# xyfJASON/ctrlora

Measured on NVIDIA B200. Metric: ddim_steps_per_sec, higher is better.
Workload: dtype fp16 (fp32 accumulate)

## Files before the change

### ctrlora_b200/_lib.py

```python
import ctypes as C
import os

_LIB_PATH = os.path.join(os.path.dirname(os.path.abspath(__file__)), "lib", "libctrlora_b200.so")
_lib = None

c_void_p, c_int, c_ll, c_float = C.c_void_p, C.c_int, C.c_longlong, C.c_float


class GemmArgs(C.Structure):
    _fields_ = [
        ("a", c_void_p), ("a_b", c_int), ("a_h", c_int), ("a_w", c_int), ("a_c", c_int), ("a_ld", c_ll),
        ("w", c_void_p), ("kh", c_int), ("kw", c_int), ("pad", c_int),
        ("a2", c_void_p), ("a2_c", c_int), ("a2_ld", c_ll), ("w2", c_void_p),
        ("n", c_int), ("block_n", c_int), ("geglu", c_int),
        ("out", c_void_p * 3), ("seg_width", c_int), ("transposed", c_int * 3),
        ("ldc", c_int), ("out_f32", c_int),
        ("bias", c_void_p), ("rowbias", c_void_p), ("rows_per_img", c_int), ("rowbias_ld", c_int),
        ("residual", c_void_p), ("ldr", c_int), ("residual_f32", c_int), ("out_scale", c_float),
        ("head_dim", c_int), ("tok_pad", c_int), ("bf16", c_int),
        ("split_k", c_int), ("splitk_ws", c_void_p), ("splitk_ws_bytes", c_ll),
        ("splitk_counters", c_void_p), ("splitk_counters_len", c_int),
        ("dup_out", c_void_p), ("dup_ld", c_int), ("force_single_cta", c_int),
    ]

# ... 16 lines not shown
_STATUS = {1: "bad argument", 2: "CUDA error", 3: "tensor-map encode error", 4: "unsupported"}


def lib_path():
    return _LIB_PATH


def load():
    global _lib
    if _lib is None:
        if not os.path.exists(_LIB_PATH):
            raise CtrloraError(
                f"{_LIB_PATH} is missing: run `python -m ctrlora_b200.build` (needs nvcc). "
                "ctrlora_b200 has no CPU or PyTorch fallback.")
        _lib = C.CDLL(_LIB_PATH)
        _declare(_lib)
    return _lib


_P, _I, _L, _F = c_void_p, c_int, c_ll, c_float
_ARGTYPES = {
    "ctrlora_gemm_f16": [_P, _P],
    "ctrlora_gemm_f16_simt": [_P, _P],
    "ctrlora_groupnorm_f16": [_P, _P],
    "ctrlora_layernorm_f16": [_P, _L, _P, _L, _I, _I, _P, _P, _F, _P],
    "ctrlora_attention_f16": [_P, _L, _P, _L, _P, _I, _P, _L, _P, _I, _I, _I, _I, _I, _P],
    "ctrlora_attention_bwd_f16": [_P, _L, _P, _L, _P, _L, _P, _L, _P, _L, _P, _P, _P, _L, _P, _L, _P, _L, _I, _I, _I, _I, _I, _P],
    "ctrlora_nchw_f32_to_nhwc_f16": [_P, _P, _I, _I, _I, _I, _P],
    "ctrlora_nhwc_to_nchw_f32": [_P, _I, _L, _P, _I, _I, _I, _P],
    "ctrlora_timestep_embedding": [_P, _P, _P, _I, _I, _P],
    "ctrlora_small_linear": [_P, _I, _P, _P, _P, _I, _I, _I, _I, _I, _I, _P],
    "ctrlora_upsample2x_f16": [_P, _P, _I, _I, _I, _I, _P],
    "ctrlora_im2col_s2_f16": [_P, _P, _I, _I, _I, _I, _P],
    "ctrlora_cast_transpose_f32_to_f16": [_P, _P, _L, _I, _I, _P],
    "ctrlora_transpose_f16": [_P, _P, _L, _I, _I, _P],
    "ctrlora_conv_dgrad_weight_f16": [_P, _P, _I, _I, _I, _P],
    "ctrlora_set_sm_limit": [_I],
    "ctrlora_ddim_update": [_P, _P, _P, _P, _P, _P, _P, _I, _I, _F, _F, _F, _F, _F, _F, _P],
    "ctrlora_wgrad_tn_f16": [_P, _L, _P, _L, _I, _I, _I, _P, _L, _F, _F, _P, _L, _P],
    "ctrlora_groupnorm_bwd_f16": [_P, _P, _P, _P, _L, _F, _P, _L, _F, _P, _L, _P, _P, _P],
    "ctrlora_layernorm_bwd_f16": [_P, _L, _P, _L, _P, _L, _I, _I, _P, _F, _P, _P, _P, _L, _P],
    "ctrlora_geglu_fwd_f16": [_P, _P, _L, _I, _P],
    "ctrlora_geglu_bwd_f16": [_P, _P, _P, _L, _I, _P],
    "ctrlora_colsum": [_P, _I, _L, _L, _I, _F, _P, _P],
    "ctrlora_image_colsum_f16": [_P, _L, _I, _I, _I, _P, _L, _P],
    "ctrlora_upsample2x_bwd_f16": [_P, _P, _I, _I, _I, _I, _P],
# ... 18 lines not shown


def _declare(lib):
    lib.ctrlora_abi_version.restype = c_int
    lib.ctrlora_last_cuda_error.restype = C.c_char_p
    for name in EXPORTS:
        fn = getattr(lib, name)
        if name not in ("ctrlora_abi_version", "ctrlora_last_cuda_error"):
            fn.restype = c_int
            fn.argtypes = _ARGTYPES[name]


def check(status, what):
    if status != 0:
        err = load().ctrlora_last_cuda_error()
        raise CtrloraError(f"{what} failed: {_STATUS.get(status, status)} ({err.decode() if err else ''})")


EXPORTS = [
    "ctrlora_abi_version",
    "ctrlora_last_cuda_error",
    "ctrlora_gemm_f16",
    "ctrlora_gemm_f16_simt",
    "ctrlora_groupnorm_f16",
    "ctrlora_layernorm_f16",
    "ctrlora_attention_f16",
    "ctrlora_nchw_f32_to_nhwc_f16",
    "ctrlora_nhwc_to_nchw_f32",
    "ctrlora_timestep_embedding",
    "ctrlora_small_linear",
    "ctrlora_upsample2x_f16",
    "ctrlora_im2col_s2_f16",
    "ctrlora_cast_transpose_f32_to_f16",
    "ctrlora_transpose_f16",
    "ctrlora_conv_dgrad_weight_f16",
    "ctrlora_set_sm_limit",
    "ctrlora_ddim_update",
    "ctrlora_wgrad_tn_f16",
    "ctrlora_attention_bwd_f16",
    "ctrlora_groupnorm_bwd_f16",
    "ctrlora_layernorm_bwd_f16",
    "ctrlora_geglu_fwd_f16",
    "ctrlora_geglu_bwd_f16",
    "ctrlora_colsum",
    "ctrlora_image_colsum_f16",
    "ctrlora_upsample2x_bwd_f16",
# ... 19 lines not shown
```

### ctrlora_b200/csrc/common.cuh

```cuda
#pragma once
#include <cuda.h>
#include <cuda_runtime.h>
#include <cuda_fp16.h>
#include <stdint.h>
#include <stdio.h>
#include <stdlib.h>
#include <string.h>

#define CTRLORA_OK 0
#define CTRLORA_ERR_ARG 1
#define CTRLORA_ERR_CUDA 2
#define CTRLORA_ERR_TMAP 3
#define CTRLORA_ERR_UNSUPPORTED 4

namespace ctrl {

__device__ __forceinline__ uint32_t smem_u32(const void* p) {
    return static_cast<uint32_t>(__cvta_generic_to_shared(p));
}

__device__ __forceinline__ void mbar_init(uint64_t* bar, uint32_t count) {
    asm volatile("mbarrier.init.shared::cta.b64 [%0], %1;" ::"r"(smem_u32(bar)), "r"(count) : "memory");
}
__device__ __forceinline__ void fence_barrier_init() {
// ... 238 lines not shown
    const float e = fast_exp2(-z * z);
    const float t = fast_rcp(fmaf(0.27273706287f, fabsf(z), 1.0f));
    float poly = fmaf(1.061405429f, t, -1.453152027f);
    poly = fmaf(poly, t, 1.421413741f);
    poly = fmaf(poly, t, -0.284496736f);
    poly = fmaf(poly, t, 0.254829592f);
    const float w = poly * t * e;
    return fmaf(-0.5f * fabsf(x), w, fmaxf(x, 0.0f));
}

}

namespace ctrl {
constexpr uint32_t kPeerBitMask = 0xFEFFFFFFu;

__device__ __forceinline__ uint32_t cluster_ctarank() {
    uint32_t r;
    asm volatile("mov.u32 %0, %%cluster_ctarank;" : "=r"(r));
    return r;
}
__device__ __forceinline__ void cluster_sync_all() {
    asm volatile("barrier.cluster.arrive.release.aligned;\n\tbarrier.cluster.wait.acquire.aligned;" ::: "memory");
}
__device__ __forceinline__ void tma_load_3d_2cta(void* dst, const CUtensorMap* m, uint64_t* bar, int c0, int c1, int c2) {
    asm volatile(
        "cp.async.bulk.tensor.3d.cta_group::2.shared::cluster.global.mbarrier::complete_tx::bytes [%0], [%1, {%3, %4, %5}], [%2];" ::"r"(
            smem_u32(dst)),
        "l"(reinterpret_cast<uint64_t>(m)), "r"(smem_u32(bar) & kPeerBitMask), "r"(c0), "r"(c1), "r"(c2)
        : "memory");
}
__device__ __forceinline__ void tma_load_4d_2cta(void* dst, const CUtensorMap* m, uint64_t* bar, int c0, int c1, int c2, int c3) {
    asm volatile(
        "cp.async.bulk.tensor.4d.cta_group::2.shared::cluster.global.mbarrier::complete_tx::bytes [%0], [%1, {%3, %4, %5, %6}], "
        "[%2];" ::"r"(smem_u32(dst)),
        "l"(reinterpret_cast<uint64_t>(m)), "r"(smem_u32(bar) & kPeerBitMask), "r"(c0), "r"(c1), "r"(c2), "r"(c3)
        : "memory");
}
__device__ __forceinline__ void umma_f16_2cta(uint32_t d_tmem, uint64_t a_desc, uint64_t b_desc, uint32_t idesc, uint32_t accumulate) {
    asm volatile(
        "{\n\t.reg .pred p;\n\t"
        "setp.ne.b32 p, %4, 0;\n\t"
        "tcgen05.mma.cta_group::2.kind::f16 [%0], %1, %2, %3, p;\n\t}" ::"r"(d_tmem),
        "l"(a_desc), "l"(b_desc), "r"(idesc), "r"(accumulate)
        : "memory");
}
__device__ __forceinline__ void umma_commit_2cta(uint64_t* bar) {
// ... 165 lines not shown
```

### ctrlora_b200/csrc/gemm_sm100.cu

```cuda
#include "gemm_sm100.cuh"
#include "ctrlora_b200.h"
#include <stdio.h>
#include <string.h>

namespace ctrl {

__device__ __forceinline__ uint32_t pack_h2(float a, float b) {
    __half2 h = __floats2half2_rn(a, b);
    return *reinterpret_cast<uint32_t*>(&h);
}

template <bool GEGLU>
__device__ __forceinline__ void epilogue_chunk(const GemmKParams& p, float* v, const float* g, int c, int bn_out, int n0,
                                               bool row_ok, long long m, int img, int tok, const float* sb,
                                               const uint4* rpre = nullptr) {
    const int nbase = n0 + c;
    const bool full_chunk = (c + 32 <= bn_out) && (nbase + 32 <= p.N);
#pragma unroll
    for (int q = 0; q < 8; ++q) {
        const float4 b4 = lds128f(smem_u32(sb + c + 4 * q));
        v[4 * q] += b4.x; v[4 * q + 1] += b4.y; v[4 * q + 2] += b4.z; v[4 * q + 3] += b4.w;
    }
    if (GEGLU) {
#pragma unroll
// ... 94 lines not shown
            for (int j = 0; j < 32; ++j)
                if (c + j < bn_out && nbase + j < p.N) o[j] = __float2half_rn(v[j]);
        }
    }
}

__device__ __forceinline__ void red_add_v4(float* addr, float a, float b, float c, float d) {
    asm volatile("red.global.add.v4.f32 [%0], {%1, %2, %3, %4};" ::"l"(addr), "f"(a), "f"(b), "f"(c), "f"(d) : "memory");
}

template <bool GEGLU, bool PAIR>
__global__ void __launch_bounds__(GEMM_THREADS, 1)
gemm_tcgen05_kernel(const __grid_constant__ CUtensorMap tmA, const __grid_constant__ CUtensorMap tmB,
                    const __grid_constant__ CUtensorMap tmA2, const __grid_constant__ CUtensorMap tmB2,
                    const __grid_constant__ GemmEpiMaps em, const __grid_constant__ GemmKParams p) {
    extern __shared__ uint8_t smem_raw[];
    uint8_t* smem = reinterpret_cast<uint8_t*>((reinterpret_cast<uintptr_t>(smem_raw) + 1023) & ~uintptr_t(1023));
    uint64_t* bars = reinterpret_cast<uint64_t*>(smem + GEMM_SMEM_DATA);
    uint64_t* full = bars;
    uint64_t* empty = bars + GEMM_MAX_STAGES;
    uint64_t* tfull = bars + 2 * GEMM_MAX_STAGES;
    uint64_t* tempty = bars + 2 * GEMM_MAX_STAGES + 2;
    uint32_t* tmem_ptr = reinterpret_cast<uint32_t*>(bars + 2 * GEMM_MAX_STAGES + 4);
    volatile int* last_flag = reinterpret_cast<volatile int*>(bars + 2 * GEMM_MAX_STAGES + 5);
    uint64_t* rfull = bars + 2 * GEMM_MAX_STAGES + 6;
    uint64_t* rempty = bars + 2 * GEMM_MAX_STAGES + 8;
    float* sbias_all = reinterpret_cast<float*>(smem + GEMM_SMEM_DATA + 512);

    pdl_launch_dependents();
    const int warp = uniform_warp_idx();
    const int lane = threadIdx.x & 31;
    const int nstages = p.stages;
    const uint32_t rank = PAIR ? cluster_ctarank() : 0u;
    const bool leader = rank == 0;

    if (warp == 0 && lane == 0) {
        tma_prefetch_desc(&tmA);
        tma_prefetch_desc(&tmB);
        if (p.epi_tma) {
            tma_prefetch_desc(&em.out[0][0]);
            tma_prefetch_desc(&em.out[0][1]);
            if (p.epi_res) { tma_prefetch_desc(&em.res[0]); tma_prefetch_desc(&em.res[1]); }
        }
        if (p.kchunks2 > 0) {
            tma_prefetch_desc(&tmA2);
            tma_prefetch_desc(&tmB2);
        }
    }
    if (warp == 1 && lane == 0) {
        for (int i = 0; i < nstages; ++i) {
            mbar_init(&full[i], 1);
            mbar_init(&empty[i], 1);
        }
        for (int i = 0; i < 2; ++i) {
            mbar_init(&tfull[i], 1);
            mbar_init(&tempty[i], PAIR ? 2 * GEMM_EPI_WARPS : GEMM_EPI_WARPS);
            mbar_init(&rfull[i], 1);
// ... 2 lines not shown
        fence_barrier_init();
    }
    if (warp == 2) {
        if (PAIR) tmem_alloc_2cta(tmem_ptr, 512);
        else tmem_alloc(tmem_ptr, 512);
    }
    tc_fence_before();
    __syncthreads();
    if (PAIR) cluster_sync_all();
    tc_fence_after();
    const uint32_t tmem_base = *tmem_ptr;
    pdl_wait();

    const int m_tiles = p.tiles_w * p.tiles_h * p.tiles_b;
    const int m_units = PAIR ? (m_tiles + 1) / 2 : m_tiles;
    const int total_tiles = m_units * p.n_tiles * p.splits;
    const int tile_first = PAIR ? static_cast<int>(blockIdx.x >> 1) : static_cast<int>(blockIdx.x);
    const int tile_stride = PAIR ? static_cast<int>(gridDim.x >> 1) : static_cast<int>(gridDim.x);
    const int main_iters = p.taps * p.kchunks;
    const int k_iters = main_iters + p.kchunks2;
    const int bn_out = GEGLU ? (p.BN >> 1) : p.BN;

    auto decode = [&](int tile, int& mt, int& ks, int& nt) {
        mt = tile % m_units;
        if (PAIR) mt = 2 * mt + static_cast<int>(rank);
        const int rest = tile / m_units;
        ks = rest % p.splits;
        nt = rest / p.splits;
    };

    if (warp == 0) {
        {
            const uint32_t tx_bytes = PAIR ? 2 * (GEMM_A_BYTES + (p.BN >> 1) * 128) : GEMM_A_BYTES + p.BN * 128;
            const int kchunks = p.kchunks, kw = p.kw, pad = p.pad, kps = p.kiters_per_split;
            const uint32_t stage_bytes = static_cast<uint32_t>(p.stage_bytes);
            const uint32_t smem0 = smem_u32(smem), full0 = smem_u32(full), empty0 = smem_u32(empty);
            const uint32_t gate_off = GEMM_A_BYTES + static_cast<uint32_t>(bn_out) * 128;
            const uint32_t rfull0 = smem_u32(rfull), rempty0 = smem_u32(rempty);
            int stage = 0, rbuf = 0;
            uint32_t phase = 0, a_dst = smem0, fb = full0, eb = empty0, rphase = 0;
            for (int tile = tile_first; tile < total_tiles; tile += tile_stride) {
                int mt, ks, nt;
                decode(tile, mt, ks, nt);
                const int tw = mt % p.tiles_w, th = (mt / p.tiles_w) % p.tiles_h, tb = mt / (p.tiles_w * p.tiles_h);
                const int w0 = tw * p.bw - pad, h0 = th * p.bh - pad, b0 = tb * p.nb, n0 = nt * bn_out;
                const int brow = !PAIR ? n0 : GEGLU ? (leader ? n0 : p.N + n0) : n0 + static_cast<int>(rank) * (p.BN >> 1);
// ... 32 lines not shown
                        tma_load_3d_a<PAIR>(a_dst + GEMM_A_BYTES, &tmB2, fb, c0, 0, brow);
                    }
                    __syncwarp();
                    c0 += GEMM_BK;
                    a_dst += stage_bytes; fb += 8; eb += 8;
                    if (++stage == nstages) { stage = 0; phase ^= 1; a_dst = smem0; fb = full0; eb = empty0; }
                }
                if (p.epi_res) {
                    mbar_wait_a(rempty0 + 8 * rbuf, rphase ^ 1);
                    if (elect_one()) {
                        const uint32_t rb = rfull0 + 8 * rbuf;
                        const uint32_t dst = smem0 + p.epi_off + rbuf * p.epi_buf_bytes;
                        mbar_expect_tx_a(rb, GEMM_BM * bn_out * 2);
                        for (int b = 0; b < p.epi_nfull; ++b)
                            tma_load_4d_a<false>(dst + b * 16384, &em.res[0], rb, n0 + 64 * b, w0 + pad, h0 + pad, b0);
                        if (p.epi_tail)
                            tma_load_4d_a<false>(dst + p.epi_nfull * 16384, &em.res[1], rb, n0 + 64 * p.epi_nfull, w0 + pad, h0 + pad, b0);
                    }
                    __syncwarp();
                    if (++rbuf == p.epi_nbuf) { rbuf = 0; rphase ^= 1; }
                }
            }
        }
    } else if (warp == 1) {
        if (leader) {
            const int kps = p.kiters_per_split;
            const uint32_t idesc = p.idesc;
            const uint32_t full0 = smem_u32(full), empty0 = smem_u32(empty), tfull0 = smem_u32(tfull), tempty0 = smem_u32(tempty);
            const uint64_t a_desc0 = umma_desc_kmajor_sw128(smem_u32(smem));
            const uint64_t b_desc0 = umma_desc_kmajor_sw128(smem_u32(smem) + GEMM_A_BYTES);
            const uint32_t stage_step = static_cast<uint32_t>(p.stage_bytes) >> 4;
            int stage = 0;
            uint32_t phase = 0, fb = full0, eb = empty0, desc_off = 0;
            int acc = 0;
            uint32_t acc_phase = 0;
            for (int tile = tile_first; tile < total_tiles; tile += tile_stride) {
                const int ks = (tile / m_units) % p.splits;
                const int it0 = ks * kps, it1 = min(k_iters, it0 + kps);
                mbar_wait_a(tempty0 + 8 * acc, acc_phase ^ 1);
                tc_fence_after();
                const uint32_t d_tmem = tmem_base + acc * 256;
                uint32_t accum = 0;
                for (int it = it0; it < it1; ++it) {
                    mbar_wait_a(fb, phase);
                    tc_fence_after();
                    const uint64_t a_desc = a_desc0 + desc_off, b_desc = b_desc0 + desc_off;
                    if (elect_one()) {
#pragma unroll
                        for (int k = 0; k < GEMM_BK / 16; ++k) {
                            if (PAIR) umma_f16_2cta(d_tmem, a_desc + 2 * k, b_desc + 2 * k, idesc, (accum | k) ? 1u : 0u);
                            else umma_f16(d_tmem, a_desc + 2 * k, b_desc + 2 * k, idesc, (accum | k) ? 1u : 0u);
                        }
                        umma_commit_a<PAIR>(eb);
                        if (it + 1 == it1) umma_commit_a<PAIR>(tfull0 + 8 * acc);
                    }
                    __syncwarp();
                    accum = 1;
                    fb += 8; eb += 8; desc_off += stage_step;
                    if (++stage == nstages) { stage = 0; phase ^= 1; fb = full0; eb = empty0; desc_off = 0; }
                }
                acc ^= 1;
                if (acc == 0) acc_phase ^= 1;
            }
        }
    } else {
        const int lane_grp = warp & 3;
        const int half = (warp - 2) >> 2;
        const int r = lane_grp * 32 + lane;
        const int iw = r % p.bw, ih = (r / p.bw) % p.bh, ib = r / (p.bw * p.bh);
        int acc = 0;
        uint32_t acc_phase = 0;
        int tile_iter = 0;
        for (int tile = tile_first; tile < total_tiles; tile += tile_stride, ++tile_iter) {
            int mt, ks, nt;
            decode(tile, mt, ks, nt);
            const int tw = mt % p.tiles_w, th = (mt / p.tiles_w) % p.tiles_h, tb = mt / (p.tiles_w * p.tiles_h);
            const int gw = tw * p.bw + iw, gh = th * p.bh + ih, gb = tb * p.nb + ib;
            const bool row_ok = gw < p.W && gh < p.H && gb < p.Bn;
            const long long m = (static_cast<long long>(gb) * p.H + gh) * p.W + gw;
            const int n0 = nt * bn_out;
            const int img = row_ok ? static_cast<int>(m / p.rows_per_img) : 0;
            const int tok = row_ok ? static_cast<int>(m % p.rows_per_img) : 0;

            float* sb = sbias_all + (tile_iter & 1) * 512;
            {
                const int e = threadIdx.x - 64;
                float bv = 0.f, bg = 0.f;
// ... 127 lines not shown
                for (int i = 0; i < 4; ++i) {
                    const int c = 32 * half + 64 * i;
                    if (c >= bn_out) break;
                    uint32_t raw[32];
                    float v[32], g[GEGLU ? 32 : 1];
                    tmem_ld_32x32(t_row + c, raw);
                    if (GEGLU) {
                        uint32_t graw[32];
                        tmem_ld_32x32(t_row + bn_out + c, graw);
                        tmem_ld_wait();
#pragma unroll
                        for (int j = 0; j < 32; ++j) g[j] = __uint_as_float(graw[j]);
                    } else {
                        tmem_ld_wait();
                    }
#pragma unroll
                    for (int j = 0; j < 32; ++j) v[j] = __uint_as_float(raw[j]);
                    epilogue_chunk<GEGLU>(p, v, g, c, bn_out, n0, row_ok, m, img, tok, sb);
                }
                tc_fence_before();
                __syncwarp();
                if (lane == 0) { if (PAIR) mbar_arrive_leader(&tempty[acc]); else mbar_arrive(&tempty[acc]); }
            } else {
                const int tile_mn = nt * m_tiles + mt;
                const long long slice = static_cast<long long>(GEMM_BM) * p.BN;
                float* wrow0 = p.ws + static_cast<long long>(tile_mn) * p.splits * slice + static_cast<long long>(r) * 4;
                float* wrow = wrow0 + ks * slice;
                auto wofs = [](int col) { return static_cast<long long>(col >> 2) * (GEMM_BM * 4); };
                for (int c = 32 * half; c < p.BN; c += 64) {
                    uint32_t raw[32];
                    tmem_ld_32x32(t_row + c, raw);
                    tmem_ld_wait();
#pragma unroll
                    for (int q = 0; q < 8; ++q)
                        if (c + 4 * q < p.BN)
                            __stcg(reinterpret_cast<float4*>(wrow + wofs(c + 4 * q)),
                                   make_float4(__uint_as_float(raw[4 * q]), __uint_as_float(raw[4 * q + 1]),
                                               __uint_as_float(raw[4 * q + 2]), __uint_as_float(raw[4 * q + 3])));
                }
                tc_fence_before();
                __syncwarp();
                if (lane == 0) mbar_arrive(&tempty[acc]);
                __threadfence();
                asm volatile("bar.sync 1, %0;" ::"n"(32 * GEMM_EPI_WARPS) : "memory");
                if (warp == 2 && lane == 0) {
                    const unsigned int old = atomicAdd(&p.counters[tile_mn], 1u);
                    const int last = (old == static_cast<unsigned int>(p.splits - 1));
                    if (last) p.counters[tile_mn] = 0;
                    *last_flag = last;
                }
                asm volatile("bar.sync 1, %0;" ::"n"(32 * GEMM_EPI_WARPS) : "memory");
                const int is_last = *last_flag;
                if (is_last) {
                    __threadfence();
                    for (int c = 32 * half; c < bn_out; c += 64) {
                        float v[32], g[32];
#pragma unroll
                        for (int q = 0; q < 8; ++q) {
                            float4 t4 = make_float4(0.f, 0.f, 0.f, 0.f), g4 = t4;
                            if (c + 4 * q < bn_out) {
                                for (int sl = 0; sl < p.splits; ++sl) {
                                    const float4 x4 = __ldcg(reinterpret_cast<const float4*>(wrow0 + sl * slice + wofs(c + 4 * q)));
                                    t4.x += x4.x; t4.y += x4.y; t4.z += x4.z; t4.w += x4.w;
                                    if (GEGLU) {
                                        const float4 y4 = __ldcg(reinterpret_cast<const float4*>(wrow0 + sl * slice + wofs(bn_out + c + 4 * q)));
                                        g4.x += y4.x; g4.y += y4.y; g4.z += y4.z; g4.w += y4.w;
                                    }
                                }
                            }
                            v[4 * q] = t4.x; v[4 * q + 1] = t4.y; v[4 * q + 2] = t4.z; v[4 * q + 3] = t4.w;
                            g[4 * q] = g4.x; g[4 * q + 1] = g4.y; g[4 * q + 2] = g4.z; g[4 * q + 3] = g4.w;
                        }
                        epilogue_chunk<GEGLU>(p, v, g, c, bn_out, n0, row_ok, m, img, tok, sb);
                    }
                }
                asm volatile("bar.sync 1, %0;" ::"n"(32 * GEMM_EPI_WARPS) : "memory");
            }
            acc ^= 1;
            if (acc == 0) acc_phase ^= 1;
        }
        if (p.epi_tma && lane == 0) bulk_wait_group<0>();
    }
    tc_fence_before();
    __syncthreads();
    if (PAIR) cluster_sync_all();
    if (warp == 2) {
        __syncwarp();
        if (PAIR) tmem_dealloc_2cta(tmem_base, 512);
        else tmem_dealloc(tmem_base, 512);
    }
}

typedef CUresult (*PFN_tmapEncodeTiled)(CUtensorMap*, CUtensorMapDataType, cuuint32_t, void*, const cuuint64_t*,
                                        const cuuint64_t*, const cuuint32_t*, const cuuint32_t*, CUtensorMapInterleave,
                                        CUtensorMapSwizzle, CUtensorMapL2promotion, CUtensorMapFloatOOBfill);

PFN_tmapEncodeTiled get_tmap_encoder() {
    static PFN_tmapEncodeTiled fn = nullptr;
    if (!fn) {
// ... 24 lines not shown
    CUresult r = enc(map, CU_TENSOR_MAP_DATA_TYPE_FLOAT16, rank, const_cast<void*>(base), gdim, gstr, bx, es,
                     CU_TENSOR_MAP_INTERLEAVE_NONE, swz, CU_TENSOR_MAP_L2_PROMOTION_L2_256B,
                     CU_TENSOR_MAP_FLOAT_OOB_FILL_NONE);
    if (r != CUDA_SUCCESS) {
        fprintf(stderr, "ctrlora: cuTensorMapEncodeTiled failed (%d) rank %d dims", (int)r, rank);
        for (int i = 0; i < rank; ++i) fprintf(stderr, " %llu", (unsigned long long)dims[i]);
        fprintf(stderr, " box");
        for (int i = 0; i < rank; ++i) fprintf(stderr, " %u", box[i]);
        fprintf(stderr, "\n");
        return CTRLORA_ERR_TMAP;
    }
    return CTRLORA_OK;
}

static int pow2_floor(int x) {
    int p = 1;
    while (p * 2 <= x) p *= 2;
    return p;
}

static int g_num_sms = 0;
static int g_sm_limit = 0;
static bool g_attr_set = false;

}

using namespace ctrl;

extern "C" int ctrlora_gemm_f16(const ctrlora_gemm_args* a, void* stream_) {
    cudaStream_t stream = reinterpret_cast<cudaStream_t>(stream_);
    if (!a || !a->a || !a->w || !a->out[0]) return CTRLORA_ERR_ARG;
    if (a->a_c % 8 != 0 || a->a_ld % 8 != 0) return CTRLORA_ERR_ARG;
    if (a->kh != a->kw || (a->kh != 1 && a->kh != 3)) return CTRLORA_ERR_UNSUPPORTED;
    if (a->bf16) return CTRLORA_ERR_UNSUPPORTED;
    GemmKParams p;
    memset(&p, 0, sizeof(p));
    p.W = a->a_w; p.H = a->a_h; p.Bn = a->a_b;
    p.bw = pow2_floor(p.W < 128 ? p.W : 128);
    p.bh = pow2_floor(p.H < 128 / p.bw ? p.H : 128 / p.bw);
    p.nb = 128 / (p.bw * p.bh);
    p.tiles_w = (p.W + p.bw - 1) / p.bw;
    p.tiles_h = (p.H + p.bh - 1) / p.bh;
    p.tiles_b = (p.Bn + p.nb - 1) / p.nb;
    p.N = a->n;
    p.taps = a->kh * a->kw; p.kw = a->kw; p.pad = a->pad;
    p.kchunks = (a->a_c + GEMM_BK - 1) / GEMM_BK;
// ... 16 lines not shown
    const bool pair_ok = pair_env && pair_shape && g_num_sms >= 2 && a->force_single_cta == 0;
    static int epi_env = -1;
    if (epi_env < 0) {
        const char* e = getenv("CTRLORA_GEMM_EPI");
        epi_env = (e && e[0] == '0') ? 0 : (e && e[0] == '2') ? 2 : 1;
    }
    bool epi_legal = !a->out_f32 && a->split_k <= 1 && a->ldc % 8 == 0 && (reinterpret_cast<uintptr_t>(a->out[0]) & 15) == 0 &&
                     (!a->residual || (!a->residual_f32 && a->ldr % 8 == 0 && (reinterpret_cast<uintptr_t>(a->residual) & 15) == 0));
    if (a->seg_width > 0) {
        const int nseg = (a->n + a->seg_width - 1) / a->seg_width;
        if (a->residual || nseg > 3 || a->seg_width % 8 != 0) epi_legal = false;
        for (int i = 0; i < nseg && i < 3; ++i)
            if (!a->transposed[i] && (!a->out[i] || (reinterpret_cast<uintptr_t>(a->out[i]) & 15) != 0)) epi_legal = false;
        if (a->dup_out && ((reinterpret_cast<uintptr_t>(a->dup_out) & 15) != 0 || a->dup_ld % 8 != 0)) epi_legal = false;
    } else if (a->transposed[0] || a->dup_out) {
        epi_legal = false;
    }
    static int epi_kmax = -1;
    if (epi_kmax < 0) {
        const char* e = getenv("CTRLORA_GEMM_EPI_KMAX");
        epi_kmax = e ? atoi(e) : 32;
    }
    const bool epi_wanted = epi_legal && (epi_env == 2 || (epi_env == 1 && k_iters <= epi_kmax));
    int bn_out = a->block_n, splits = a->split_k > 0 ? a->split_k : 1;
    if (bn_out <= 0) {
        double best_cost = -1;
        const int max_out = p.geglu ? 128 : 256;
        static const int split_cands[] = {1, 2, 3, 4, 6, 8, 12, 16};
        for (int cand = max_out; cand >= 16; cand -= 16) {
            if (a->seg_width > 0 && a->seg_width % cand != 0) continue;
            if (epi_wanted && cand % 32 != 0) continue;
            const int bnt = p.geglu ? 2 * cand : cand;
            const int nt = (p.N + cand - 1) / cand;
            const long tiles_mn = (long)m_tiles * nt;
            const double waste = (double)nt * cand / p.N;
            for (int si = 0; si < 8; ++si) {
                int S = split_cands[si];
                if (a->split_k > 0) { if (si > 0) break; S = a->split_k; }
                if (S > 1) {
                    if (a->split_k <= 0) break;
                    if (!a->splitk_ws || !a->splitk_counters) break;
                    if ((long long)tiles_mn * S * GEMM_BM * bnt * 4 > a->splitk_ws_bytes || tiles_mn > a->splitk_counters_len) break;
                    if (a->seg_width > 0 && a->transposed[0] + a->transposed[1] + a->transposed[2] > 0 && false) break;
                }
                const int kps = (k_iters + S - 1) / S;
                if (S > 1 && kps < 4 && a->split_k <= 0) break;
                const int s_eff = (k_iters + kps - 1) / kps;
                const bool cpair = pair_ok && s_eff == 1 && bnt % 32 == 0;
                const long tiles = cpair ? (long)((m_tiles + 1) / 2) * nt : tiles_mn * s_eff;
                const long slots = cpair ? g_num_sms / 2 : g_num_sms;
                const long waves = (tiles + slots - 1) / slots;
                const double t_mma = kps * 4.0 * (bnt / 2 > 32 ? bnt / 2 : 32);
                const double t_load = kps * (double)(GEMM_A_BYTES + (cpair ? bnt / 2 : bnt) * 128) / 69.0;
                const double t_epi = (cand / 32 + 1) * 350.0;
                double t_tile = (t_mma > t_load ? t_mma : t_load);
                if (t_epi > t_tile) t_tile = t_epi;
                t_tile += 600.0;
                if (s_eff > 1) t_tile += bnt * 12.0 + t_epi;
                const double cost = waves * t_tile * (0.5 + 0.5 * waste);
                if (best_cost < 0 || cost < best_cost) { best_cost = cost; bn_out = cand; splits = s_eff; }
            }
        }
    }
    if (bn_out % 16 != 0 || bn_out < 16 || bn_out > (p.geglu ? 128 : 256)) return CTRLORA_ERR_ARG;
    if (a->seg_width > 0 && a->seg_width % bn_out != 0) return CTRLORA_ERR_ARG;
    p.BN = p.geglu ? 2 * bn_out : bn_out;
    p.n_tiles = (p.N + bn_out - 1) / bn_out;
    p.kiters_per_split = (k_iters + splits - 1) / splits;
    p.splits = (k_iters + p.kiters_per_split - 1) / p.kiters_per_split;
    if (p.splits > 1) {
        const long long tiles_mn = (long long)m_tiles * p.n_tiles;
        if (!a->splitk_ws || !a->splitk_counters || tiles_mn * p.splits * GEMM_BM * p.BN * 4 > a->splitk_ws_bytes ||
            tiles_mn > a->splitk_counters_len)
            return CTRLORA_ERR_ARG;
        p.ws = a->splitk_ws;
        p.counters = a->splitk_counters;
    }
    const bool pair = pair_ok && p.splits == 1 && (p.BN % 32 == 0);
    const int b_rows = pair ? p.BN / 2 : p.BN;
    p.stage_bytes = GEMM_A_BYTES + ((b_rows * 128 + 1023) / 1024) * 1024;
    int ring_bytes = GEMM_SMEM_DATA;
    {
        if (epi_wanted && p.splits == 1 && bn_out % 32 == 0) {
            const int nfull = bn_out / 64, tail = (bn_out % 64) ? 1 : 0;
            const int buf_bytes = nfull * 16384 + tail * 8192;
            int nbuf = 2;
            if ((GEMM_SMEM_DATA - 2 * buf_bytes) / p.stage_bytes < 3) nbuf = 1;
            static int nbuf_env = -1;
            if (nbuf_env < 0) {
                const char* e = getenv("CTRLORA_GEMM_EPI_NBUF");
                nbuf_env = e ? atoi(e) : 0;
            }
            if (nbuf_env == 1) nbuf = 1;
            if ((GEMM_SMEM_DATA - nbuf * buf_bytes) / p.stage_bytes >= 3) {
                p.epi_tma = 1; p.epi_nbuf = nbuf; p.epi_res = a->residual ? 1 : 0;
                p.epi_nfull = nfull; p.epi_tail = tail; p.epi_buf_bytes = buf_bytes;
                p.epi_off = GEMM_SMEM_DATA - nbuf * buf_bytes;
                ring_bytes = p.epi_off;
            }
        }
// ... 59 lines not shown
            box[0] = 32;
            return make_tmap_f16_sw(&dst[1], base, 4, dims, str, box, CU_TENSOR_MAP_SWIZZLE_64B);
        };
        if (a->seg_width > 0) {
            const int nseg = (p.N + a->seg_width - 1) / a->seg_width;
            for (int i = 0; i < nseg; ++i) {
                if (a->transposed[i]) continue;
                int rc = pair_of(em.out[i], a->out[i], a->ldc, a->seg_width, sw, sh, sb);
                if (rc) return rc;
            }
            if (a->dup_out) {
                int rc = pair_of(em.dup, a->dup_out, a->dup_ld, a->seg_width, sw, sh, sb);
                if (rc) return rc;
            }
        } else {
            int rc = pair_of(em.out[0], a->out[0], a->ldc, p.N, sw, sh, sb);
            if (rc) return rc;
        }
        if (p.epi_res) {
            int rc = pair_of(em.res, a->residual, a->ldr, p.N, p.bw, p.bh, p.nb);
            if (rc) return rc;
        }
    }
    if (!g_attr_set) {
        if (cudaFuncSetAttribute(gemm_tcgen05_kernel<false, false>, cudaFuncAttributeMaxDynamicSharedMemorySize, GEMM_SMEM_BYTES) != cudaSuccess ||
            cudaFuncSetAttribute(gemm_tcgen05_kernel<true, false>, cudaFuncAttributeMaxDynamicSharedMemorySize, GEMM_SMEM_BYTES) != cudaSuccess ||
            cudaFuncSetAttribute(gemm_tcgen05_kernel<false, true>, cudaFuncAttributeMaxDynamicSharedMemorySize, GEMM_SMEM_BYTES) != cudaSuccess ||
            cudaFuncSetAttribute(gemm_tcgen05_kernel<true, true>, cudaFuncAttributeMaxDynamicSharedMemorySize, GEMM_SMEM_BYTES) != cudaSuccess)
            return CTRLORA_ERR_CUDA;
        g_attr_set = true;
    }
    cudaError_t lrc;
    if (pair) {
        const int units = ((m_tiles + 1) / 2) * p.n_tiles;
        int clusters = (g_sm_limit > 0 && g_sm_limit < g_num_sms ? g_sm_limit : g_num_sms) / 2;
        if (units < clusters) clusters = units;
        const dim3 grid2(2 * clusters), block(GEMM_THREADS);
        lrc = p.geglu ? launch_cluster(gemm_tcgen05_kernel<true, true>, grid2, block, (size_t)GEMM_SMEM_BYTES, stream, 2u, tmA, tmB, tmA2, tmB2, em, p)
                      : launch_cluster(gemm_tcgen05_kernel<false, true>, grid2, block, (size_t)GEMM_SMEM_BYTES, stream, 2u, tmA, tmB, tmA2, tmB2, em, p);
    } else {
        const int total = m_tiles * p.n_tiles * p.splits;
        const int sms_avail = g_sm_limit > 0 && g_sm_limit < g_num_sms ? g_sm_limit : g_num_sms;
        const int grid = total < sms_avail ? total : sms_avail;
        lrc = p.geglu ? launch_pdl(gemm_tcgen05_kernel<true, false>, dim3(grid), dim3(GEMM_THREADS), (size_t)GEMM_SMEM_BYTES,
                                   stream, tmA, tmB, tmA2, tmB2, em, p)
                      : launch_pdl(gemm_tcgen05_kernel<false, false>, dim3(grid), dim3(GEMM_THREADS), (size_t)GEMM_SMEM_BYTES,
                                   stream, tmA, tmB, tmA2, tmB2, em, p);
    }
    if (lrc != cudaSuccess) return CTRLORA_ERR_CUDA;
    return cudaGetLastError() == cudaSuccess ? CTRLORA_OK : CTRLORA_ERR_CUDA;
}

extern "C" int ctrlora_set_sm_limit(int limit) {
    if (limit < 0) return CTRLORA_ERR_ARG;
    g_sm_limit = limit;
    return CTRLORA_OK;
}
```

### ctrlora_b200/csrc/gemm_sm100.cuh

```cuda
#pragma once
#include "common.cuh"

namespace ctrl {

constexpr int GEMM_BM = 128;
constexpr int GEMM_BK = 64;
constexpr int GEMM_MAX_STAGES = 10;
constexpr int GEMM_A_BYTES = GEMM_BM * GEMM_BK * 2;
constexpr int GEMM_EPI_WARPS = 8;
constexpr int GEMM_THREADS = 64 + 32 * GEMM_EPI_WARPS;
constexpr int GEMM_SMEM_DATA = 216 * 1024;
constexpr int GEMM_SMEM_BYTES = GEMM_SMEM_DATA + 1024  + 512  + 4096 ;

struct GemmEpiMaps {
    CUtensorMap out[3][2];
    CUtensorMap dup[2];
    CUtensorMap res[2];
};

struct GemmKParams {
    int W, H, Bn;
    int bw, bh, nb;
    int tiles_w, tiles_h, tiles_b;
    int N;
    int BN;
    int n_tiles;
    int taps, kw, pad;
    int kchunks;
    int kchunks2;
    int geglu;
    int stages, stage_bytes;
    int splits, kiters_per_split;
    float* ws;
    unsigned int* counters;
    uint32_t idesc;
    void* out[3];
    int seg_width;
    int transposed[3];
    int ldc;
    int out_f32;
    const float* bias;
    const float* rowbias;
    int rows_per_img;
    int rowbias_ld;
    int residual_f32;
    const __half* residual;
    int ldr;
    float out_scale;
    int head_dim, tok_pad;
    __half* dup_out;
    int dup_ld;
    int bf16;
    int epi_tma, epi_nbuf, epi_res;
    int epi_off, epi_buf_bytes;
    int epi_nfull, epi_tail;
};

// ... 2 lines not shown
```

### include/ctrlora_b200.h

```cpp
#ifndef CTRLORA_B200_H
#define CTRLORA_B200_H

#ifdef __cplusplus
extern "C" {
#endif

#define CTRLORA_ABI_VERSION 2

#define CTRLORA_STATUS_OK 0
#define CTRLORA_STATUS_BAD_ARGUMENT 1
#define CTRLORA_STATUS_CUDA_ERROR 2
#define CTRLORA_STATUS_TENSORMAP_ERROR 3
#define CTRLORA_STATUS_UNSUPPORTED 4

int ctrlora_abi_version(void);
const char* ctrlora_last_cuda_error(void);

int ctrlora_memset_zero(void* ptr, long long bytes, void* stream);

typedef struct ctrlora_gemm_args {
    const void* a;
    int a_b, a_h, a_w, a_c;
    long long a_ld;
    const void* w;
// ... 11 lines not shown
    int ldc;
    int out_f32;
    const float* bias;
    const float* rowbias;
    int rows_per_img;
    int rowbias_ld;
    const void* residual;
    int ldr;
    int residual_f32;
    float out_scale;
    int head_dim, tok_pad;
    int bf16;
    int split_k;
    float* splitk_ws;
    long long splitk_ws_bytes;
    unsigned int* splitk_counters;
    int splitk_counters_len;
    void* dup_out;
    int dup_ld;
    int force_single_cta;
} ctrlora_gemm_args;

int ctrlora_gemm_f16(const ctrlora_gemm_args* args, void* stream);

int ctrlora_gemm_f16_simt(const ctrlora_gemm_args* args, void* stream);

typedef struct ctrlora_groupnorm_args {
    const void* x1; const void* add1; float add1_scale; int c1; long long ld1;
    const void* x2; const void* add2; float add2_scale; int c2; long long ld2;
    int batch, hw, groups;
    const float* gamma; const float* beta; float eps; int silu;
    void* y;
    void* raw_out;
    void* stats_ws;
    int stats_prezeroed;
    float* partial_ws;
    long long partial_ws_floats;
    unsigned int* partial_counters;
    int partial_counters_len;
} ctrlora_groupnorm_args;
int ctrlora_groupnorm_f16(const ctrlora_groupnorm_args* args, void* stream);

int ctrlora_layernorm_f16(const void* x, long long ldx, void* y, long long ldy, int rows, int cols,
                          const float* gamma, const float* beta, float eps, void* stream);

int ctrlora_attention_f16(const void* q, long long ldq, const void* k, long long ldk, const void* vt, int nk_pad,
// ... 81 lines not shown
```

Baseline: 69.35.

## Replace global-workspace split-K with cluster-based DSMEM split-K reduction

Split-K partial sums are now exchanged through distributed shared memory inside a thread-block cluster of size `splits`. Each CTA reduces its share of rows and runs the epilogue for them, replacing the global workspace with its atomic counters and last-CTA reduction. The tile heuristic now considers split-K by default, even without a caller-supplied workspace, when the MN tile count underfills the SMs and the clusters fit in occupancy. This targets small-M/N, large-K GEMMs that leave SMs idle. The cost is extra cluster barriers and launch constraints, plus a new query export for the last chosen config.

```diff
diff --git a/ctrlora_b200/_lib.py b/ctrlora_b200/_lib.py
--- a/ctrlora_b200/_lib.py
+++ b/ctrlora_b200/_lib.py
@@ -62,6 +62,7 @@
 _ARGTYPES = {
     "ctrlora_gemm_f16": [_P, _P],
     "ctrlora_gemm_f16_simt": [_P, _P],
+    "ctrlora_gemm_last_config": [_P, _P, _P],
     "ctrlora_groupnorm_f16": [_P, _P],
     "ctrlora_layernorm_f16": [_P, _L, _P, _L, _I, _I, _P, _P, _F, _P],
     "ctrlora_attention_f16": [_P, _L, _P, _L, _P, _I, _P, _L, _P, _I, _I, _I, _I, _I, _P],
@@ -126,6 +127,7 @@
     "ctrlora_last_cuda_error",
     "ctrlora_gemm_f16",
     "ctrlora_gemm_f16_simt",
+    "ctrlora_gemm_last_config",
     "ctrlora_groupnorm_f16",
     "ctrlora_layernorm_f16",
     "ctrlora_attention_f16",
diff --git a/ctrlora_b200/csrc/common.cuh b/ctrlora_b200/csrc/common.cuh
--- a/ctrlora_b200/csrc/common.cuh
+++ b/ctrlora_b200/csrc/common.cuh
@@ -284,6 +284,14 @@
 __device__ __forceinline__ void cluster_sync_all() {
     asm volatile("barrier.cluster.arrive.release.aligned;\n\tbarrier.cluster.wait.acquire.aligned;" ::: "memory");
 }
+__device__ __forceinline__ uint32_t mapa_shared(uint32_t addr, uint32_t rank) {
+    uint32_t r;
+    asm volatile("mapa.shared::cluster.u32 %0, %1, %2;" : "=r"(r) : "r"(addr), "r"(rank));
+    return r;
+}
+__device__ __forceinline__ void st_dsmem128(uint32_t cluster_addr, uint32_t a, uint32_t b, uint32_t c, uint32_t d) {
+    asm volatile("st.shared::cluster.v4.b32 [%0], {%1, %2, %3, %4};" ::"r"(cluster_addr), "r"(a), "r"(b), "r"(c), "r"(d) : "memory");
+}
 __device__ __forceinline__ void tma_load_3d_2cta(void* dst, const CUtensorMap* m, uint64_t* bar, int c0, int c1, int c2) {
     asm volatile(
         "cp.async.bulk.tensor.3d.cta_group::2.shared::cluster.global.mbarrier::complete_tx::bytes [%0], [%1, {%3, %4, %5}], [%2];" ::"r"(
diff --git a/ctrlora_b200/csrc/gemm_sm100.cu b/ctrlora_b200/csrc/gemm_sm100.cu
--- a/ctrlora_b200/csrc/gemm_sm100.cu
+++ b/ctrlora_b200/csrc/gemm_sm100.cu
@@ -140,7 +140,6 @@
     uint64_t* tfull = bars + 2 * GEMM_MAX_STAGES;
     uint64_t* tempty = bars + 2 * GEMM_MAX_STAGES + 2;
     uint32_t* tmem_ptr = reinterpret_cast<uint32_t*>(bars + 2 * GEMM_MAX_STAGES + 4);
-    volatile int* last_flag = reinterpret_cast<volatile int*>(bars + 2 * GEMM_MAX_STAGES + 5);
     uint64_t* rfull = bars + 2 * GEMM_MAX_STAGES + 6;
     uint64_t* rempty = bars + 2 * GEMM_MAX_STAGES + 8;
     float* sbias_all = reinterpret_cast<float*>(smem + GEMM_SMEM_DATA + 512);
@@ -151,6 +150,7 @@
     const int nstages = p.stages;
     const uint32_t rank = PAIR ? cluster_ctarank() : 0u;
     const bool leader = rank == 0;
+    const bool csplit = !PAIR && p.splits > 1;
 
     if (warp == 0 && lane == 0) {
         tma_prefetch_desc(&tmA);
@@ -199,6 +199,13 @@
     const int bn_out = GEGLU ? (p.BN >> 1) : p.BN;
 
     auto decode = [&](int tile, int& mt, int& ks, int& nt) {
+        if (csplit) {
+            ks = tile % p.splits;
+            const int t = tile / p.splits;
+            mt = t % m_tiles;
+            nt = t / m_tiles;
+            return;
+        }
         mt = tile % m_units;
         if (PAIR) mt = 2 * mt + static_cast<int>(rank);
         const int rest = tile / m_units;
@@ -277,6 +284,7 @@
                 }
             }
         }
+        if (csplit) { cluster_sync_all(); cluster_sync_all(); }
     } else if (warp == 1) {
         if (leader) {
             const int kps = p.kiters_per_split;
@@ -290,7 +298,8 @@
             int acc = 0;
             uint32_t acc_phase = 0;
             for (int tile = tile_first; tile < total_tiles; tile += tile_stride) {
-                const int ks = (tile / m_units) % p.splits;
+                int mt, ks, nt;
+                decode(tile, mt, ks, nt);
                 const int it0 = ks * kps, it1 = min(k_iters, it0 + kps);
                 mbar_wait_a(tempty0 + 8 * acc, acc_phase ^ 1);
                 tc_fence_after();
@@ -318,6 +327,7 @@
                 if (acc == 0) acc_phase ^= 1;
             }
         }
+        if (csplit) { cluster_sync_all(); cluster_sync_all(); }
     } else {
         const int lane_grp = warp & 3;
         const int half = (warp - 2) >> 2;
@@ -491,59 +501,53 @@
                 __syncwarp();
                 if (lane == 0) { if (PAIR) mbar_arrive_leader(&tempty[acc]); else mbar_arrive(&tempty[acc]); }
             } else {
-                const int tile_mn = nt * m_tiles + mt;
-                const long long slice = static_cast<long long>(GEMM_BM) * p.BN;
-                float* wrow0 = p.ws + static_cast<long long>(tile_mn) * p.splits * slice + static_cast<long long>(r) * 4;
-                float* wrow = wrow0 + ks * slice;
-                auto wofs = [](int col) { return static_cast<long long>(col >> 2) * (GEMM_BM * 4); };
-                for (int c = 32 * half; c < p.BN; c += 64) {
-                    uint32_t raw[32];
-                    tmem_ld_32x32(t_row + c, raw);
-                    tmem_ld_wait();
-#pragma unroll
-                    for (int q = 0; q < 8; ++q)
-                        if (c + 4 * q < p.BN)
-                            __stcg(reinterpret_cast<float4*>(wrow + wofs(c + 4 * q)),
-                                   make_float4(__uint_as_float(raw[4 * q]), __uint_as_float(raw[4 * q + 1]),
-                                               __uint_as_float(raw[4 * q + 2]), __uint_as_float(raw[4 * q + 3])));
+                constexpr int QW = GEGLU ? 16 : 8;
+                const int nchunks = (bn_out + 31) / 32, items = 4 * nchunks;
+                const uint32_t recv = smem_u32(smem);
+                cluster_sync_all();
+                for (int ci = half; ci < nchunks; ci += 2) {
+                    const int c = 32 * ci, i = lane_grp + 4 * ci;
+                    const uint32_t dst = mapa_shared(recv + (((i / p.splits) * p.splits + ks) * QW * 512 + lane * 16),
+                                                     static_cast<uint32_t>(i % p.splits));
+                    for (int part = 0; part < (GEGLU ? 2 : 1); ++part) {
+                        uint32_t raw[32];
+                        tmem_ld_32x32(t_row + part * bn_out + c, raw);
+                        tmem_ld_wait();
+#pragma unroll
+                        for (int q = 0; q < 8; ++q)
+                            st_dsmem128(dst + (8 * part + q) * 512, raw[4 * q], raw[4 * q + 1], raw[4 * q + 2], raw[4 * q + 3]);
+                    }
                 }
                 tc_fence_before();
                 __syncwarp();
                 if (lane == 0) mbar_arrive(&tempty[acc]);
-                __threadfence();
-                asm volatile("bar.sync 1, %0;" ::"n"(32 * GEMM_EPI_WARPS) : "memory");
-                if (warp == 2 && lane == 0) {
-                    const unsigned int old = atomicAdd(&p.counters[tile_mn], 1u);
-                    const int last = (old == static_cast<unsigned int>(p.splits - 1));
-                    if (last) p.counters[tile_mn] = 0;
-                    *last_flag = last;
-                }
-                asm volatile("bar.sync 1, %0;" ::"n"(32 * GEMM_EPI_WARPS) : "memory");
-                const int is_last = *last_flag;
-                if (is_last) {
-                    __threadfence();
-                    for (int c = 32 * half; c < bn_out; c += 64) {
-                        float v[32], g[32];
+                cluster_sync_all();
+                for (int i = ks + p.splits * (warp - 2); i < items; i += p.splits * GEMM_EPI_WARPS) {
+                    const int rr = 32 * (i & 3) + lane, c = 32 * (i >> 2);
+                    const int jw = rr % p.bw, jh = (rr / p.bw) % p.bh, jb = rr / (p.bw * p.bh);
+                    const int qw = tw * p.bw + jw, qh = th * p.bh + jh, qb = tb * p.nb + jb;
+                    const bool qrow_ok = qw < p.W && qh < p.H && qb < p.Bn;
+                    const long long qm = (static_cast<long long>(qb) * p.H + qh) * p.W + qw;
+                    const int qimg = qrow_ok ? static_cast<int>(qm / p.rows_per_img) : 0;
+                    const int qtok = qrow_ok ? static_cast<int>(qm % p.rows_per_img) : 0;
+                    float v[32], g[GEGLU ? 32 : 1];
+#pragma unroll
+                    for (int j = 0; j < 32; ++j) { v[j] = 0.f; if (GEGLU) g[j] = 0.f; }
+                    const uint32_t src0 = recv + (i / p.splits) * p.splits * QW * 512 + lane * 16;
+                    for (int s = 0; s < p.splits; ++s) {
+                        const uint32_t src = src0 + s * QW * 512;
 #pragma unroll
                         for (int q = 0; q < 8; ++q) {
-                            float4 t4 = make_float4(0.f, 0.f, 0.f, 0.f), g4 = t4;
-                            if (c + 4 * q < bn_out) {
-                                for (int sl = 0; sl < p.splits; ++sl) {
-                                    const float4 x4 = __ldcg(reinterpret_cast<const float4*>(wrow0 + sl * slice + wofs(c + 4 * q)));
-                                    t4.x += x4.x; t4.y += x4.y; t4.z += x4.z; t4.w += x4.w;
-                                    if (GEGLU) {
-                                        const float4 y4 = __ldcg(reinterpret_cast<const float4*>(wrow0 + sl * slice + wofs(bn_out + c + 4 * q)));
-                                        g4.x += y4.x; g4.y += y4.y; g4.z += y4.z; g4.w += y4.w;
-                                    }
-                                }
+                            const float4 x4 = lds128f(src + q * 512);
+                            v[4 * q] += x4.x; v[4 * q + 1] += x4.y; v[4 * q + 2] += x4.z; v[4 * q + 3] += x4.w;
+                            if (GEGLU) {
+                                const float4 y4 = lds128f(src + (8 + q) * 512);
+                                g[4 * q] += y4.x; g[4 * q + 1] += y4.y; g[4 * q + 2] += y4.z; g[4 * q + 3] += y4.w;
                             }
-                            v[4 * q] = t4.x; v[4 * q + 1] = t4.y; v[4 * q + 2] = t4.z; v[4 * q + 3] = t4.w;
-                            g[4 * q] = g4.x; g[4 * q + 1] = g4.y; g[4 * q + 2] = g4.z; g[4 * q + 3] = g4.w;
                         }
-                        epilogue_chunk<GEGLU>(p, v, g, c, bn_out, n0, row_ok, m, img, tok, sb);
-                    }
-                }
-                asm volatile("bar.sync 1, %0;" ::"n"(32 * GEMM_EPI_WARPS) : "memory");
+                    }
+                    epilogue_chunk<GEGLU>(p, v, g, c, bn_out, n0, qrow_ok, qm, qimg, qtok, sb);
+                }
             }
             acc ^= 1;
             if (acc == 0) acc_phase ^= 1;
@@ -614,6 +618,33 @@
 static int g_num_sms = 0;
 static int g_sm_limit = 0;
 static bool g_attr_set = false;
+static thread_local int g_last_bn = 0, g_last_splits = 0, g_last_pair = 0;
+
+static int max_active_clusters(int S) {
+    static int cache[GEMM_MAX_SPLIT + 1] = {0};
+    if (S < 1 || S > GEMM_MAX_SPLIT) return 0;
+    if (cache[S] == 0) {
+        cudaLaunchConfig_t cfg;
+        memset(&cfg, 0, sizeof(cfg));
+        cfg.gridDim = dim3(S);
+        cfg.blockDim = dim3(GEMM_THREADS);
+        cfg.dynamicSmemBytes = GEMM_SMEM_BYTES;
+        cudaLaunchAttribute at[1];
+        at[0].id = cudaLaunchAttributeClusterDimension;
+        at[0].val.clusterDim.x = S;
+        at[0].val.clusterDim.y = 1;
+        at[0].val.clusterDim.z = 1;
+        cfg.attrs = at;
+        cfg.numAttrs = 1;
+        int n = 0;
+        if (cudaOccupancyMaxActiveClusters(&n, gemm_tcgen05_kernel<false, false>, &cfg) != cudaSuccess) {
+            (void)cudaGetLastError();
+            n = 0;
+        }
+        cache[S] = n > 0 ? n : -1;
+    }
+    return cache[S] > 0 ? cache[S] : 0;
+}
 
 }
 
@@ -676,11 +707,25 @@
         epi_kmax = e ? atoi(e) : 32;
     }
     const bool epi_wanted = epi_legal && (epi_env == 2 || (epi_env == 1 && k_iters <= epi_kmax));
-    int bn_out = a->block_n, splits = a->split_k > 0 ? a->split_k : 1;
+    if (!g_attr_set) {
+        if (cudaFuncSetAttribute(gemm_tcgen05_kernel<false, false>, cudaFuncAttributeMaxDynamicSharedMemorySize, GEMM_SMEM_BYTES) != cudaSuccess ||
+            cudaFuncSetAttribute(gemm_tcgen05_kernel<true, false>, cudaFuncAttributeMaxDynamicSharedMemorySize, GEMM_SMEM_BYTES) != cudaSuccess ||
+            cudaFuncSetAttribute(gemm_tcgen05_kernel<false, true>, cudaFuncAttributeMaxDynamicSharedMemorySize, GEMM_SMEM_BYTES) != cudaSuccess ||
+            cudaFuncSetAttribute(gemm_tcgen05_kernel<true, true>, cudaFuncAttributeMaxDynamicSharedMemorySize, GEMM_SMEM_BYTES) != cudaSuccess)
+            return CTRLORA_ERR_CUDA;
+        g_attr_set = true;
+    }
+    static int csplit_env = -1;
+    if (csplit_env < 0) {
+        const char* e = getenv("CTRLORA_GEMM_CLUSTER_SPLIT");
+        csplit_env = (e && e[0] == '0') ? 0 : 1;
+    }
+    const int sms_avail = g_sm_limit > 0 && g_sm_limit < g_num_sms ? g_sm_limit : g_num_sms;
+    int bn_out = a->block_n;
+    int splits = a->split_k > 1 ? (a->split_k < GEMM_MAX_SPLIT ? a->split_k : GEMM_MAX_SPLIT) : 1;
     if (bn_out <= 0) {
         double best_cost = -1;
         const int max_out = p.geglu ? 128 : 256;
-        static const int split_cands[] = {1, 2, 3, 4, 6, 8, 12, 16};
         for (int cand = max_out; cand >= 16; cand -= 16) {
             if (a->seg_width > 0 && a->seg_width % cand != 0) continue;
             if (epi_wanted && cand % 32 != 0) continue;
@@ -688,18 +733,13 @@
             const int nt = (p.N + cand - 1) / cand;
             const long tiles_mn = (long)m_tiles * nt;
             const double waste = (double)nt * cand / p.N;
-            for (int si = 0; si < 8; ++si) {
-                int S = split_cands[si];
-                if (a->split_k > 0) { if (si > 0) break; S = a->split_k; }
-                if (S > 1) {
-                    if (a->split_k <= 0) break;
-                    if (!a->splitk_ws || !a->splitk_counters) break;
-                    if ((long long)tiles_mn * S * GEMM_BM * bnt * 4 > a->splitk_ws_bytes || tiles_mn > a->splitk_counters_len) break;
-                    if (a->seg_width > 0 && a->transposed[0] + a->transposed[1] + a->transposed[2] > 0 && false) break;
-                }
+            for (int S = 1; S <= GEMM_MAX_SPLIT; ++S) {
+                if (a->split_k > 1 ? S != splits : (S > 1 && (a->split_k == 1 || !csplit_env))) continue;
                 const int kps = (k_iters + S - 1) / S;
-                if (S > 1 && kps < 4 && a->split_k <= 0) break;
                 const int s_eff = (k_iters + kps - 1) / kps;
+                if (S > 1 && a->split_k <= 0 &&
+                    (s_eff != S || kps < 4 || tiles_mn >= sms_avail || tiles_mn * S > sms_avail || tiles_mn > max_active_clusters(S)))
+                    continue;
                 const bool cpair = pair_ok && s_eff == 1 && bnt % 32 == 0;
                 const long tiles = cpair ? (long)((m_tiles + 1) / 2) * nt : tiles_mn * s_eff;
                 const long slots = cpair ? g_num_sms / 2 : g_num_sms;
@@ -708,9 +748,13 @@
                 const double t_load = kps * (double)(GEMM_A_BYTES + (cpair ? bnt / 2 : bnt) * 128) / 69.0;
                 const double t_epi = (cand / 32 + 1) * 350.0;
                 double t_tile = (t_mma > t_load ? t_mma : t_load);
-                if (t_epi > t_tile) t_tile = t_epi;
-                t_tile += 600.0;
-                if (s_eff > 1) t_tile += bnt * 12.0 + t_epi;
+                if (s_eff == 1) {
+                    if (t_epi > t_tile) t_tile = t_epi;
+                    t_tile += 600.0;
+                } else {
+                    const double t_load_c = kps * (double)(GEMM_A_BYTES + bnt * 128) / 100.0;
+                    t_tile = (t_mma > t_load_c ? t_mma : t_load_c) + 600.0 + 1000.0 + bnt * 36.0 + t_epi / s_eff;
+                }
                 const double cost = waves * t_tile * (0.5 + 0.5 * waste);
                 if (best_cost < 0 || cost < best_cost) { best_cost = cost; bn_out = cand; splits = s_eff; }
             }
@@ -722,14 +766,6 @@
     p.n_tiles = (p.N + bn_out - 1) / bn_out;
     p.kiters_per_split = (k_iters + splits - 1) / splits;
     p.splits = (k_iters + p.kiters_per_split - 1) / p.kiters_per_split;
-    if (p.splits > 1) {
-        const long long tiles_mn = (long long)m_tiles * p.n_tiles;
-        if (!a->splitk_ws || !a->splitk_counters || tiles_mn * p.splits * GEMM_BM * p.BN * 4 > a->splitk_ws_bytes ||
-            tiles_mn > a->splitk_counters_len)
-            return CTRLORA_ERR_ARG;
-        p.ws = a->splitk_ws;
-        p.counters = a->splitk_counters;
-    }
     const bool pair = pair_ok && p.splits == 1 && (p.BN % 32 == 0);
     const int b_rows = pair ? p.BN / 2 : p.BN;
     p.stage_bytes = GEMM_A_BYTES + ((b_rows * 128 + 1023) / 1024) * 1024;
@@ -835,14 +871,6 @@
             if (rc) return rc;
         }
     }
-    if (!g_attr_set) {
-        if (cudaFuncSetAttribute(gemm_tcgen05_kernel<false, false>, cudaFuncAttributeMaxDynamicSharedMemorySize, GEMM_SMEM_BYTES) != cudaSuccess ||
-            cudaFuncSetAttribute(gemm_tcgen05_kernel<true, false>, cudaFuncAttributeMaxDynamicSharedMemorySize, GEMM_SMEM_BYTES) != cudaSuccess ||
-            cudaFuncSetAttribute(gemm_tcgen05_kernel<false, true>, cudaFuncAttributeMaxDynamicSharedMemorySize, GEMM_SMEM_BYTES) != cudaSuccess ||
-            cudaFuncSetAttribute(gemm_tcgen05_kernel<true, true>, cudaFuncAttributeMaxDynamicSharedMemorySize, GEMM_SMEM_BYTES) != cudaSuccess)
-            return CTRLORA_ERR_CUDA;
-        g_attr_set = true;
-    }
     cudaError_t lrc;
     if (pair) {
         const int units = ((m_tiles + 1) / 2) * p.n_tiles;
@@ -851,9 +879,13 @@
         const dim3 grid2(2 * clusters), block(GEMM_THREADS);
         lrc = p.geglu ? launch_cluster(gemm_tcgen05_kernel<true, true>, grid2, block, (size_t)GEMM_SMEM_BYTES, stream, 2u, tmA, tmB, tmA2, tmB2, em, p)
                       : launch_cluster(gemm_tcgen05_kernel<false, true>, grid2, block, (size_t)GEMM_SMEM_BYTES, stream, 2u, tmA, tmB, tmA2, tmB2, em, p);
+    } else if (p.splits > 1) {
+        const dim3 gridc(m_tiles * p.n_tiles * p.splits), block(GEMM_THREADS);
+        const unsigned cl = static_cast<unsigned>(p.splits);
+        lrc = p.geglu ? launch_cluster_pdl(gemm_tcgen05_kernel<true, false>, gridc, block, (size_t)GEMM_SMEM_BYTES, stream, cl, tmA, tmB, tmA2, tmB2, em, p)
+                      : launch_cluster_pdl(gemm_tcgen05_kernel<false, false>, gridc, block, (size_t)GEMM_SMEM_BYTES, stream, cl, tmA, tmB, tmA2, tmB2, em, p);
     } else {
-        const int total = m_tiles * p.n_tiles * p.splits;
-        const int sms_avail = g_sm_limit > 0 && g_sm_limit < g_num_sms ? g_sm_limit : g_num_sms;
+        const int total = m_tiles * p.n_tiles;
         const int grid = total < sms_avail ? total : sms_avail;
         lrc = p.geglu ? launch_pdl(gemm_tcgen05_kernel<true, false>, dim3(grid), dim3(GEMM_THREADS), (size_t)GEMM_SMEM_BYTES,
                                    stream, tmA, tmB, tmA2, tmB2, em, p)
@@ -861,7 +893,15 @@
                                    stream, tmA, tmB, tmA2, tmB2, em, p);
     }
     if (lrc != cudaSuccess) return CTRLORA_ERR_CUDA;
-    return cudaGetLastError() == cudaSuccess ? CTRLORA_OK : CTRLORA_ERR_CUDA;
+    if (cudaGetLastError() != cudaSuccess) return CTRLORA_ERR_CUDA;
+    g_last_bn = bn_out; g_last_splits = p.splits; g_last_pair = pair ? 1 : 0;
+    return CTRLORA_OK;
+}
+
+extern "C" int ctrlora_gemm_last_config(int* block_n, int* split_k, int* pair) {
+    if (!block_n || !split_k || !pair) return CTRLORA_ERR_ARG;
+    *block_n = g_last_bn; *split_k = g_last_splits; *pair = g_last_pair;
+    return CTRLORA_OK;
 }
 
 extern "C" int ctrlora_set_sm_limit(int limit) {
diff --git a/ctrlora_b200/csrc/gemm_sm100.cuh b/ctrlora_b200/csrc/gemm_sm100.cuh
--- a/ctrlora_b200/csrc/gemm_sm100.cuh
+++ b/ctrlora_b200/csrc/gemm_sm100.cuh
@@ -6,6 +6,7 @@
 constexpr int GEMM_BM = 128;
 constexpr int GEMM_BK = 64;
 constexpr int GEMM_MAX_STAGES = 10;
+constexpr int GEMM_MAX_SPLIT = 8;
 constexpr int GEMM_A_BYTES = GEMM_BM * GEMM_BK * 2;
 constexpr int GEMM_EPI_WARPS = 8;
 constexpr int GEMM_THREADS = 64 + 32 * GEMM_EPI_WARPS;
@@ -31,8 +32,6 @@
     int geglu;
     int stages, stage_bytes;
     int splits, kiters_per_split;
-    float* ws;
-    unsigned int* counters;
     uint32_t idesc;
     void* out[3];
     int seg_width;
diff --git a/include/ctrlora_b200.h b/include/ctrlora_b200.h
--- a/include/ctrlora_b200.h
+++ b/include/ctrlora_b200.h
@@ -57,6 +57,8 @@
 } ctrlora_gemm_args;
 
 int ctrlora_gemm_f16(const ctrlora_gemm_args* args, void* stream);
+
+int ctrlora_gemm_last_config(int* block_n, int* split_k, int* pair);
 
 int ctrlora_gemm_f16_simt(const ctrlora_gemm_args* args, void* stream);
 
```

Result: faster. 70.22 (median of 6 runs) (+1.3%).
